# hynkis/Python-MPC

Measured on NVIDIA B200. Metric: lateral-MPC QP solves/sec (batch 65536, H=20), higher is better.
Workload: dtype f64

## Files before the change

### python-mpc_b200/csrc/mpc_b200.cu

```cuda
#include "shape_ops.cuh"
#include "models.cuh"

static thread_local std::string g_err;
static int env_int(const char* name, int dflt) { const char* v = std::getenv(name); return v ? std::atoi(v) : dflt; }
namespace mpcb_rt {
std::atomic<long long> g_launches{0};
std::atomic<int> g_opt_tma{std::getenv("MPCB_NO_TMA") ? 0 : 1};
std::atomic<int> g_opt_retile{std::getenv("MPCB_NO_RETILE") ? 0 : 1};
std::atomic<int> g_opt_cert{std::getenv("MPCB_NO_CERT") ? 0 : 1};
std::atomic<int> g_opt_dense{std::getenv("MPCB_NO_DENSE") ? 0 : 1};
std::atomic<int> g_opt_cta{std::getenv("MPCB_NO_CTA") ? 0 : 1};
std::atomic<int> g_opt_warp_setup{std::getenv("MPCB_NO_WARP_SETUP") ? 0 : 1};
std::atomic<int> g_opt_retile_min{env_int("MPCB_RETILE_MIN_BATCH", 4096)};
std::atomic<int> g_opt_fwd_rhs{std::getenv("MPCB_NO_FWD_RHS") ? 0 : 1};
int fail(int code, const std::string& msg) {
    g_err = msg;
    return code;
}
}

static const ShapeOps** registry(int* count_out, const ShapeOps* add) {
    static const ShapeOps* table[64];
    static int count = 0;
    if (add && count < 64) table[count++] = add;
    if (count_out) *count_out = count;
    return table;
}
namespace mpcb_rt {
void register_shape_ops(const ShapeOps* ops) { registry(nullptr, ops); }
}
static const ShapeOps* find_ops(int nx, int nu, int slack, int dtype) {
    int n = 0;
    const ShapeOps** t = registry(&n, nullptr);
    for (int i = 0; i < n; ++i)
        if (t[i]->nx == nx && t[i]->nu == nu && (t[i]->slack != 0) == (slack != 0) && t[i]->dtype == dtype) return t[i];
    return nullptr;
}
static const ShapeOps* ops_of(const mpcb_solver* s) {
    return find_ops(s->prob.nx, s->prob.nu, s->prob.slack, s->prob.dtype);
}

static bool is_big(double v) { return !(std::fabs(v) < kOsqpInfty * kMinScaling * 1e-6); }
static int problem_has_inf_bounds(const mpcb_problem& q) {
    for (int i = 0; i < q.nx; ++i) if (is_big(q.xmin[i]) || is_big(q.xmax[i])) return 1;
    for (int i = 0; i < q.nu; ++i) if (is_big(q.umin[i]) || is_big(q.umax[i])) return 1;
    return 0;
}

static bool shape_supported(int nx, int nu, int slack) { return find_ops(nx, nu, slack, MPCB_F64) != nullptr; }


const char* mpcb_last_error(void) { return g_err.c_str(); }
int mpcb_version(void) { return 100; }
long long mpcb_launch_count(void) { return g_launches.load(); }

int mpcb_set_option(const char* name, int value) {
    if (!name) return fail(MPCB_E_ARG, "null option name");
    const std::string n(name);
    if (n == "tma") g_opt_tma = value != 0;
    else if (n == "retile") g_opt_retile = value != 0;
    else if (n == "certificates") g_opt_cert = value != 0;
    else if (n == "dense") g_opt_dense = value != 0;
    else if (n == "warp_setup") g_opt_warp_setup = value != 0;
    else if (n == "cta") g_opt_cta = value < 0 ? 0 : (value > 2 ? 2 : value);
    else if (n == "retile_min_batch") g_opt_retile_min = value;
    else if (n == "fwd_rhs") g_opt_fwd_rhs = value != 0;
    else return fail(MPCB_E_ARG, "unknown option: " + n);
    return 0;
}

void mpcb_default_settings(mpcb_settings* s) {
    s->rho = 0.1; s->sigma = 1e-6; s->alpha = 1.6; s->eps_abs = 1e-3; s->eps_rel = 1e-3;
    s->eps_prim_inf = 1e-4; s->eps_dual_inf = 1e-4; s->max_iter = 4000; s->scaling = 10;
    s->check_termination = 25; s->warm_start = 1;
}

static int check_settings(const mpcb_settings* o) {
    if (!(o->rho > 0) || !(o->sigma > 0) || !(o->alpha > 0 && o->alpha < 2) || o->max_iter <= 0 ||
        o->scaling < 0 || o->check_termination < 0 || o->eps_abs < 0 || o->eps_rel < 0 ||
        (o->eps_abs == 0 && o->eps_rel == 0))
        return fail(MPCB_E_ARG, "invalid settings (rho, sigma > 0; 0 < alpha < 2; max_iter > 0; eps >= 0, not both 0)");
    return 0;
}

int mpcb_create(const mpcb_problem* prob, const mpcb_settings* settings, int capacity, mpcb_solver** out) {
    if (!prob || !out || capacity <= 0) return fail(MPCB_E_ARG, "null problem / non-positive capacity");
    if (prob->horizon < 1) return fail(MPCB_E_ARG, "horizon must be >= 1");
    if (prob->dtype != MPCB_F32 && prob->dtype != MPCB_F64) return fail(MPCB_E_ARG, "dtype must be MPCB_F32 or MPCB_F64");
    if (!shape_supported(prob->nx, prob->nu, prob->slack))
        return fail(MPCB_E_ARG, "unsupported (nx, nu, slack) combination");
    for (int i = 0; i < prob->nx; ++i)
        if (prob->xmin[i] > prob->xmax[i]) return fail(MPCB_E_ARG, "lower bound must be lower than or equal to upper bound");
    for (int i = 0; i < prob->nu; ++i)
        if (prob->umin[i] > prob->umax[i]) return fail(MPCB_E_ARG, "lower bound must be lower than or equal to upper bound");
    mpcb_settings def;
    mpcb_default_settings(&def);
    if (!settings) settings = &def;
    if (int rc = check_settings(settings)) return rc;
    mpcb_solver* s = new (std::nothrow) mpcb_solver();
    if (!s) return fail(MPCB_E_ALLOC, "out of host memory");
    s->prob = *prob; s->set = *settings; s->cap = capacity;
#ifndef MPCB_EMU
    if (cudaGetDevice(&s->dev) != cudaSuccess ||
        cudaDeviceGetAttribute(&s->dev_max_smem, cudaDevAttrMaxSharedMemoryPerBlockOptin, s->dev) != cudaSuccess ||
        cudaDeviceGetAttribute(&s->dev_sms, cudaDevAttrMultiProcessorCount, s->dev) != cudaSuccess) {
        const std::string msg = std::string("cuda device query: ") + cudaGetErrorString(cudaGetLastError());
        delete s;
        return fail(MPCB_E_CUDA, msg);
    }
#endif
    s->inf_prob = problem_has_inf_bounds(*prob);
    s->inf_bounds = s->inf_prob;
    s->esz = prob->dtype == MPCB_F32 ? 4 : 8;
    const int N = prob->horizon, nx = prob->nx, nu = prob->nu, ns = prob->slack ? nx : 0;
    s->VS = nx + ns + nu; s->CS = 2 * nx + nu; s->NW = nx + nu; s->LT = s->NW * (s->NW + 1) / 2;
    s->REC = 2 * s->VS + 2 * s->CS + s->LT + s->NW; s->HDR = 3 * nx + 1;
    s->nvar = (N + 1) * nx + N * nu + (N + 1) * ns; s->ncon = 2 * (N + 1) * nx + N * nu;
    s->ld = ((size_t)capacity + 31) / 32 * 32;
    const size_t ld = s->ld, e = s->esz, S1 = (size_t)(N + 1);
    struct { void** p; size_t n; } allocs[] = {
        {&s->rec, S1 * s->REC * ld * e}, {&s->hdr, (size_t)s->HDR * ld * e}, {&s->yrows, S1 * s->CS * ld * e},
        {&s->scr, S1 * (s->VS + s->CS) * ld * e}, {&s->scr_hdr, (size_t)nx * ld * e}, {&s->pri, ld * e},
        {&s->dua, ld * e}, {(void**)&s->iter, ld * sizeof(int)}, {(void**)&s->status, ld * sizeof(int)},
        {(void**)&s->tile_counter, 64}, {(void**)&s->surv[0], ld * sizeof(int)}, {(void**)&s->surv[1], ld * sizeof(int)},
        {(void**)&s->n_surv, 64}, {(void**)&s->tile_prog, (ld / 32 + 1) * sizeof(int)}};
    for (auto& a : allocs) {
        if (int rc = rt_malloc(a.p, a.n)) { mpcb_destroy(s); return rc; }
        s->ws_bytes += a.n;
    }
    rt_memset(s->rec, 0, S1 * s->REC * ld * e, 0);
    rt_memset(s->hdr, 0, (size_t)s->HDR * ld * e, 0);
    rt_memset(s->yrows, 0, S1 * s->CS * ld * e, 0);
    rt_memset(s->status, 0, ld * sizeof(int), 0);
    rt_sync(0);
    *out = s;
    return 0;
}

void mpcb_destroy(mpcb_solver* s) {
    if (!s) return;
    void* ptrs[] = {s->rec, s->hdr, s->yrows, s->scr, s->scr_hdr, s->pri, s->dua, s->iter, s->status, s->tile_counter,
                    s->surv[0], s->surv[1], s->n_surv, s->tile_prog, s->rec2, s->hdr2, s->yrows2,
                    s->xbox, s->xbox_alt, s->stage_in, s->stage_out, s->soa_in, s->dense_minv, s->dense_flag, s->mdl, s->mdl2};
    for (void* p : ptrs) rt_free(p);
    delete s;
}

int mpcb_set_settings(mpcb_solver* s, const mpcb_settings* o) {
    if (!s || !o) return fail(MPCB_E_ARG, "null argument");
// ... 470 lines not shown
```

### python-mpc_b200/csrc/qp_thread.cuh

```cuda
#pragma once
#include "mpc_common.h"

namespace mpcb {

MPCB_HD float msqrt(float v) { return sqrtf(v); }
MPCB_HD double msqrt(double v) { return sqrt(v); }
template <typename T> MPCB_HD T tmax(T a, T b) { return a > b ? a : b; }
template <typename T> MPCB_HD T tmin(T a, T b) { return a < b ? a : b; }
template <typename T> MPCB_HD T tabs(T a) { return a < (T)0 ? -a : a; }
template <typename T> MPCB_HD T limit_scaling(T v) {
    v = v < (T)kMinScaling ? (T)1 : v;
    return v > (T)kMaxScaling ? (T)kMaxScaling : v;
}
template <typename T> MPCB_HD T clip_infty(T v) {
    return tmin(tmax(v, (T)-kOsqpInfty), (T)kOsqpInfty);
}
template <typename T> MPCB_HD T row_rho(T l, T u, T rho, T rho_eq) {
    if (l < (T)(-kOsqpInfty * kMinScaling) && u > (T)(kOsqpInfty * kMinScaling)) return (T)kRhoMin;
    if (u - l < (T)kRhoTol) return rho_eq;
    return rho;
}
template <typename T> MPCB_HD T row_rho(bool inf_possible, T l, T u, T rho, T rho_eq) {
    if (inf_possible) return row_rho(l, u, rho, rho_eq);
    return (u - l < (T)kRhoTol) ? rho_eq : rho;
}
template <typename T> MPCB_HD T clamp_rho(T rho) {
    return tmin(tmax(rho, (T)kRhoMin), (T)kRhoMax);
}
MPCB_HD float fast_rcp(float v) { return 1.0f / v; }
MPCB_HD double fast_rcp(double v) {
#ifdef __CUDA_ARCH__
    double r;
    asm("rcp.approx.ftz.f64 %0, %1;" : "=d"(r) : "d"(v));
    r = r * (2.0 - v * r);
    r = r * (2.0 - v * r);
    return r;
#else
    return 1.0 / v;
#endif
}

MPCB_HD float fast_rsqrt(float v) { return 1.0f / sqrtf(v); }
MPCB_HD double fast_rsqrt(double v) {
#ifdef __CUDA_ARCH__
    double y;
    asm("rsqrt.approx.ftz.f64 %0, %1;" : "=d"(y) : "d"(v));
    double e = fma(-(v * y), y, 1.0);
    y = fma(0.5 * y, e, y);
    e = fma(-(v * y), y, 1.0);
    y = fma(0.5 * y, e, y);
    return y;
#else
    return 1.0 / sqrt(v);
#endif
}

template <typename T, typename L>
struct Model {
    T A[L::NX][L::NX];
    T B[L::NX][L::NU];
};
template <typename T, typename L>
MPCB_HD T model_g(const KParams<T>& p, int b, int k, int i) {
    if (!p.gd) return (T)0;
    const size_t og = p.tv ? (size_t)k * L::NX : 0;
    return p.model_bs ? p.gd[(og + i) * p.ld + b] : p.gd[og + i];
}

template <typename T, typename L>
MPCB_HD void load_model(const KParams<T>& p, int b, int k, Model<T, L>& m) {
    constexpr int NX = L::NX, NU = L::NU;
    const size_t bo = p.model_bs ? (size_t)b : 0;
    const size_t ld = p.model_bs ? p.ld : 1;
    const size_t oa = p.tv ? (size_t)k * NX * NX : 0, ob = p.tv ? (size_t)k * NX * NU : 0;
#pragma unroll
    for (int i = 0; i < NX; ++i) {
#pragma unroll
        for (int j = 0; j < NX; ++j) m.A[i][j] = p.Ad[(oa + i * NX + j) * ld + bo];
#pragma unroll
        for (int j = 0; j < NU; ++j) m.B[i][j] = p.Bd[(ob + i * NU + j) * ld + bo];
    }
}

template <typename T, typename L>
MPCB_HD void stage_box(const KParams<T>& p, int k, T* lo, T* hi) {
#pragma unroll
    for (int i = 0; i < L::NX; ++i) {
        T a = p.xbox ? p.xbox[(k * 2 + 0) * L::NX + i] : p.xmin[i];
        T c = p.xbox ? p.xbox[(k * 2 + 1) * L::NX + i] : p.xmax[i];
        lo[i] = a;
        hi[i] = c;
    }
}

template <typename T, typename L>
struct Ws {
    T* rec;
    T* hdr;
    T* y;
    T* scr;
    T* scr_hdr;
    MPCB_HD Ws(const KParams<T>& p, int b) {
        const size_t tile = (size_t)(b >> 5), lane = (size_t)(b & 31);
        const size_t S1 = (size_t)(p.N + 1);
        rec = p.rec + tile * S1 * L::REC * TILE + lane;
        hdr = p.hdr + tile * L::HDR * TILE + lane;
        y = p.yrows + tile * S1 * L::CS * TILE + lane;
        scr = p.scr + tile * S1 * (L::VS + L::CS) * TILE + lane;
        scr_hdr = p.scr_hdr + tile * L::NX * TILE + lane;
    }
    MPCB_HD T* R(int k) const { return rec + (size_t)k * L::REC * TILE; }
    MPCB_HD T* Y(int k) const { return y + (size_t)k * L::CS * TILE; }
    MPCB_HD T* S(int k) const { return scr + (size_t)k * (L::VS + L::CS) * TILE; }
};
#define MPCB_AT(ptr, e) (ptr)[(e) * TILE]

template <typename T, typename L>
struct ScaleStage {
    T Dx[L::NX], Dsl[L::NX], Du[L::NU], Ebx[L::NX], Ebu[L::NU], Edn[L::NX];
};
template <typename T, typename L>
MPCB_HD void scale_stage_update(const KParams<T>& p, const Model<T, L>& m, T c, int b, int k, const ScaleStage<T, L>& o,
                                const T* Ed_cur, const T* Dx_next, ScaleStage<T, L>& n, T* E0new, T& sumP, T& maxq) {
    constexpr int NX = L::NX, NU = L::NU, NS = L::NS;
    const bool last = (k == p.N);
    const T* Qk = last ? p.QN : p.Q;
    T colx[NX], colu[NU], rowd[NX];
#pragma unroll
    for (int j = 0; j < NX; ++j) {
        T v = c * tabs(Qk[j]) * o.Dx[j] * o.Dx[j];
        v = tmax(v, Ed_cur[j] * o.Dx[j]);
        colx[j] = tmax(v, o.Ebx[j] * o.Dx[j]);
        rowd[j] = o.Edn[j] * Dx_next[j];
    }
#pragma unroll
    for (int j = 0; j < NU; ++j) colu[j] = tmax(c * tabs(p.R[j]) * o.Du[j] * o.Du[j], o.Ebu[j] * o.Du[j]);
    if (!last) {
#pragma unroll
        for (int i = 0; i < NX; ++i) {
#pragma unroll
            for (int j = 0; j < NX; ++j) {
                const T gij = tabs(m.A[i][j]) * o.Edn[i] * o.Dx[j];
                colx[j] = tmax(colx[j], gij); rowd[i] = tmax(rowd[i], gij);
            }
#pragma unroll
            for (int j = 0; j < NU; ++j) {
                const T gij = tabs(m.B[i][j]) * o.Edn[i] * o.Du[j];
                colu[j] = tmax(colu[j], gij); rowd[i] = tmax(rowd[i], gij);
            }
        }
    }
#pragma unroll
    for (int j = 0; j < NX; ++j) {
        n.Dx[j] = o.Dx[j] * fast_rsqrt(limit_scaling(colx[j]));
        if (NS) {
            T w = tmax(c * tabs(p.W[j]) * o.Dsl[j] * o.Dsl[j], tabs(p.S[j]) * o.Ebx[j] * o.Dsl[j]);
            n.Dsl[j] = o.Dsl[j] * fast_rsqrt(limit_scaling(w));
        } else {
            n.Dsl[j] = (T)1;
        }
    }
#pragma unroll
    for (int j = 0; j < NU; ++j) n.Du[j] = last ? (T)1 : o.Du[j] * fast_rsqrt(limit_scaling(colu[j]));
    if (k == 0) {
#pragma unroll
        for (int i = 0; i < NX; ++i) {
            T v = Ed_cur[i] * o.Dx[i];
            E0new[i] = Ed_cur[i] * fast_rsqrt(limit_scaling(v));
        }
    }
#pragma unroll
    for (int i = 0; i < NX; ++i) {
        T en = (T)1;
        if (!last) en = o.Edn[i] * fast_rsqrt(limit_scaling(rowd[i]));
        n.Edn[i] = en;
        T w = o.Ebx[i] * o.Dx[i];
        if (NS) w = tmax(w, tabs(p.S[i]) * o.Ebx[i] * o.Dsl[i]);
        n.Ebx[i] = o.Ebx[i] * fast_rsqrt(limit_scaling(w));
    }
#pragma unroll
    for (int j = 0; j < NU; ++j) {
        T w = o.Ebu[j] * o.Du[j];
        n.Ebu[j] = last ? (T)1 : o.Ebu[j] * fast_rsqrt(limit_scaling(w));
    }
#pragma unroll
    for (int j = 0; j < NX; ++j) {
        sumP += c * tabs(Qk[j]) * n.Dx[j] * n.Dx[j];
        const T xr = p.Xr[((p.xr_tv ? (size_t)k * NX : 0) + j) * p.ld + b];
        maxq = tmax(maxq, tabs(c * n.Dx[j] * (-(Qk[j] * xr))));
        if (NS) sumP += c * tabs(p.W[j]) * n.Dsl[j] * n.Dsl[j];
    }
#pragma unroll
    for (int j = 0; j < NU; ++j)
        if (!last) sumP += c * tabs(p.R[j]) * n.Du[j] * n.Du[j];
}
template <typename T, typename L>
MPCB_HD T scale_cost_update(T c, T sumP, T maxq, int N) {
    T c_temp = sumP / (T)L::nvar(N);
    const T nq = limit_scaling(maxq);
    c_temp = tmax(c_temp, nq);
    c_temp = (T)1 / limit_scaling(c_temp);
    return c * c_temp;
}

template <typename T, typename L, bool ODD>
MPCB_HD void scale_pass(const KParams<T>& p, int b, const Ws<T, L>& ws, Model<T, L>& m, T& c) {
    constexpr int NX = L::NX, NU = L::NU, NS = L::NS;
    constexpr bool odd = ODD;
    const int N = p.N;
    const T* E0s = odd ? ws.scr_hdr : ws.hdr + L::H_E0 * TILE;
    T* E0d = odd ? ws.hdr + L::H_E0 * TILE : ws.scr_hdr;
    T sumP = 0, maxq = 0;
    T Ed_cur[NX];
#pragma unroll
    for (int i = 0; i < NX; ++i) Ed_cur[i] = MPCB_AT(E0s, i);
    for (int k = 0; k <= N; ++k) {
        const bool last = (k == N);
        const T* Ds = odd ? ws.S(k) : ws.R(k) + L::R_D * TILE;
        const T* Es = odd ? ws.S(k) + L::VS * TILE : ws.R(k) + L::R_E * TILE;
        T* Dd = odd ? ws.R(k) + L::R_D * TILE : ws.S(k);
        T* Ed = odd ? ws.R(k) + L::R_E * TILE : ws.S(k) + L::VS * TILE;
        const T* Dsn_ = last ? Ds : (odd ? ws.S(k + 1) : ws.R(k + 1) + L::R_D * TILE);
        if (p.tv && !last) load_model<T, L>(p, b, k, m);
        ScaleStage<T, L> o, n;
        T Dx_next[NX], E0new[NX];
#pragma unroll
        for (int i = 0; i < NX; ++i) {
            o.Dx[i] = MPCB_AT(Ds, L::OX + i);
            o.Dsl[i] = NS ? MPCB_AT(Ds, L::OS + (NS ? i : 0)) : (T)1;
            o.Ebx[i] = MPCB_AT(Es, L::OBX + i);
            o.Edn[i] = last ? (T)1 : MPCB_AT(Es, L::ODN + i);
            Dx_next[i] = last ? (T)1 : MPCB_AT(Dsn_, L::OX + i);
        }
#pragma unroll
        for (int j = 0; j < NU; ++j) {
            o.Du[j] = MPCB_AT(Ds, L::OU + j);
            o.Ebu[j] = MPCB_AT(Es, L::OBU + j);
        }
        scale_stage_update<T, L>(p, m, c, b, k, o, Ed_cur, Dx_next, n, E0new, sumP, maxq);
        if (k == 0) {
#pragma unroll
            for (int i = 0; i < NX; ++i) MPCB_AT(E0d, i) = E0new[i];
        }
#pragma unroll
        for (int i = 0; i < NX; ++i) {
            MPCB_AT(Ed, L::ODN + i) = n.Edn[i];
            MPCB_AT(Ed, L::OBX + i) = n.Ebx[i];
            MPCB_AT(Dd, L::OX + i) = n.Dx[i];
            if (NS) MPCB_AT(Dd, L::OS + (NS ? i : 0)) = n.Dsl[i];
        }
#pragma unroll
        for (int j = 0; j < NU; ++j) {
            MPCB_AT(Ed, L::OBU + j) = n.Ebu[j];
            MPCB_AT(Dd, L::OU + j) = n.Du[j];
        }
#pragma unroll
        for (int i = 0; i < NX; ++i) Ed_cur[i] = o.Edn[i];
    }
    c = scale_cost_update<T, L>(c, sumP, maxq, N);
}

template <typename T, typename L>
MPCB_HD void scale_one(const KParams<T>& p, int b) {
    constexpr int NX = L::NX;
    const int N = p.N;
    Ws<T, L> ws(p, b);
    for (int k = 0; k <= N; ++k) {
        T* R = ws.R(k);
        for (int e = 0; e < L::VS + L::CS; ++e) MPCB_AT(R, L::R_D + e) = (T)1;
    }
    for (int i = 0; i < NX; ++i) MPCB_AT(ws.hdr, L::H_E0 + i) = (T)1;
    T c = (T)1;
    Model<T, L> m;
    if (!p.tv) load_model<T, L>(p, b, 0, m);
    for (int it = 0; it < p.scaling; ++it) {
        if (it & 1) scale_pass<T, L, true>(p, b, ws, m, c);
        else scale_pass<T, L, false>(p, b, ws, m, c);
// ... 889 lines not shown
```

### python-mpc_b200/csrc/runtime.cuh

```cuda
#pragma once
#include "../../include/mpc_b200.h"
#include "mpc_common.h"
#include "qp_thread.cuh"

#include <atomic>
#include <cstdio>
#include <cstdlib>
#include <cstring>
#include <new>
#include <string>
#include <type_traits>

using namespace mpcb;

namespace mpcb_rt {
extern std::atomic<long long> g_launches;
extern std::atomic<int> g_opt_tma, g_opt_retile, g_opt_cert, g_opt_dense, g_opt_cta, g_opt_warp_setup, g_opt_retile_min, g_opt_fwd_rhs;
int fail(int code, const std::string& msg);
}
struct ShapeOps;
namespace mpcb_rt { void register_shape_ops(const ShapeOps* ops); }
using namespace mpcb_rt;

#ifndef MPCB_EMU
#include <cuda_runtime.h>
typedef cudaStream_t rt_stream;
#define RT_CHECK(expr)                                                                         \
    do {                                                                                       \
        cudaError_t e_ = (expr);                                                               \
        if (e_ != cudaSuccess)                                                                 \
            return fail(MPCB_E_CUDA, std::string(#expr) + ": " + cudaGetErrorString(e_));      \
    } while (0)
static int rt_malloc(void** p, size_t n) { RT_CHECK(cudaMalloc(p, n ? n : 1)); return 0; }
static void rt_free(void* p) { if (p) cudaFree(p); }
static int rt_memset(void* p, int v, size_t n, rt_stream s) { RT_CHECK(cudaMemsetAsync(p, v, n, s)); return 0; }
static int rt_h2d(void* d, const void* h, size_t n, rt_stream s) { RT_CHECK(cudaMemcpyAsync(d, h, n, cudaMemcpyHostToDevice, s)); return 0; }
static int rt_d2h(void* h, const void* d, size_t n, rt_stream s) { RT_CHECK(cudaMemcpyAsync(h, d, n, cudaMemcpyDeviceToHost, s)); return 0; }
static int rt_sync(rt_stream s) { RT_CHECK(cudaStreamSynchronize(s)); return 0; }
static bool debug_sync() {
    static const bool on = std::getenv("MPCB_DEBUG_SYNC") != nullptr;
    return on;
}
static int rt_launch_check(const char* what) {
    cudaError_t e = cudaGetLastError();
    if (e == cudaSuccess && debug_sync()) e = cudaDeviceSynchronize();
    if (e != cudaSuccess) return fail(MPCB_E_CUDA, std::string(what) + ": " + cudaGetErrorString(e));
    return 0;
}

#ifndef MPCB_QP_THREADS
#define MPCB_QP_THREADS 128
#endif
#ifndef MPCB_QP_MINBLOCKS
#define MPCB_QP_MINBLOCKS 2
#endif
template <typename Op, typename T, typename L>
__global__ void __launch_bounds__(MPCB_QP_THREADS, MPCB_QP_MINBLOCKS) qp_kernel(const KParams<T> p) {
    const int b = blockIdx.x * blockDim.x + threadIdx.x;
    if (b < p.B) Op::template run<T, L>(p, b);
}
template <typename Op, typename T, typename L>
static int launch_qp(const KParams<T>& p, rt_stream st) {
    const int threads = MPCB_QP_THREADS;
    qp_kernel<Op, T, L><<<(p.B + threads - 1) / threads, threads, 0, st>>>(p);
    ++g_launches;
    return rt_launch_check(Op::name());
}
template <typename F>
__global__ void __launch_bounds__(128) lambda_kernel(int n, F f) {
    const int b = blockIdx.x * blockDim.x + threadIdx.x;
    if (b < n) f(b);
}
#define MPCB_LAMBDA [=] __device__
template <typename F>
static int launch_1d(int n, rt_stream st, F f) {
    if (n <= 0) return 0;
    lambda_kernel<<<(n + 127) / 128, 128, 0, st>>>(n, f);
    ++g_launches;
    return rt_launch_check("lambda_kernel");
}
#else
typedef void* rt_stream;
static int rt_malloc(void** p, size_t n) { *p = std::malloc(n ? n : 1); return *p ? 0 : fail(MPCB_E_ALLOC, "malloc"); }
static void rt_free(void* p) { std::free(p); }
static int rt_memset(void* p, int v, size_t n, rt_stream) { std::memset(p, v, n); return 0; }
static int rt_h2d(void* d, const void* h, size_t n, rt_stream) { std::memcpy(d, h, n); return 0; }
static int rt_d2h(void* h, const void* d, size_t n, rt_stream) { std::memcpy(h, d, n); return 0; }
static int rt_sync(rt_stream) { return 0; }
template <typename Op, typename T, typename L>
static int launch_qp(const KParams<T>& p, rt_stream) {
    for (int b = 0; b < p.B; ++b) Op::template run<T, L>(p, b);
    ++g_launches;
    return 0;
}
#define MPCB_LAMBDA [=]
template <typename F>
static int launch_1d(int n, rt_stream, F f) {
    for (int b = 0; b < n; ++b) f(b);
    ++g_launches;
    return 0;
// ... 74 lines not shown
```

### python-mpc_b200/csrc/setup_warp.cuh

```cuda
#pragma once
#include "qp_thread.cuh"

#if defined(__CUDACC__) && !defined(MPCB_EMU)
namespace mpcb {

constexpr int SCALE_WARPS = 8;

template <typename T, typename L>
__global__ void __launch_bounds__(SCALE_WARPS * 32) scale_warp_kernel(const __grid_constant__ KParams<T> p) {
    constexpr int NX = L::NX, NU = L::NU, NS = L::NS;
    const int warp = threadIdx.x >> 5, k = threadIdx.x & 31;
    const int b = blockIdx.x * SCALE_WARPS + warp;
    if (b >= p.B) return;
    const int N = p.N;
    const bool stage = k <= N;
    const int kk = stage ? k : N;
    Model<T, L> m;
    load_model<T, L>(p, b, p.tv ? (kk < N ? kk : N - 1) : 0, m);
    ScaleStage<T, L> o, n;
    T E0[NX];
#pragma unroll
    for (int i = 0; i < NX; ++i) { o.Dx[i] = o.Dsl[i] = o.Ebx[i] = o.Edn[i] = (T)1; E0[i] = (T)1; }
#pragma unroll
    for (int j = 0; j < NU; ++j) { o.Du[j] = o.Ebu[j] = (T)1; }
    T c = (T)1;
    for (int it = 0; it < p.scaling; ++it) {
        T Ed_cur[NX], Dx_next[NX], E0new[NX];
#pragma unroll
        for (int i = 0; i < NX; ++i) {
            const T up = __shfl_up_sync(0xffffffffu, o.Edn[i], 1), dn = __shfl_down_sync(0xffffffffu, o.Dx[i], 1);
            Ed_cur[i] = k == 0 ? E0[i] : up;
            Dx_next[i] = k >= N ? (T)1 : dn;
            E0new[i] = E0[i];
        }
        T sumP = 0, maxq = 0;
        if (stage) scale_stage_update<T, L>(p, m, c, b, k, o, Ed_cur, Dx_next, n, E0new, sumP, maxq);
#pragma unroll
        for (int off = 16; off > 0; off >>= 1) {
            sumP += __shfl_xor_sync(0xffffffffu, sumP, off);
            maxq = tmax(maxq, __shfl_xor_sync(0xffffffffu, maxq, off));
        }
        c = scale_cost_update<T, L>(c, sumP, maxq, N);
        if (stage) o = n;
#pragma unroll
        for (int i = 0; i < NX; ++i) E0[i] = E0new[i];
    }
    if (!stage) return;
    Ws<T, L> ws(p, b);
    T* R = ws.R(k);
#pragma unroll
    for (int i = 0; i < NX; ++i) {
        MPCB_AT(R, L::R_D + L::OX + i) = o.Dx[i];
        if (NS) MPCB_AT(R, L::R_D + L::OS + (NS ? i : 0)) = o.Dsl[i];
        MPCB_AT(R, L::R_E + L::ODN + i) = o.Edn[i];
        MPCB_AT(R, L::R_E + L::OBX + i) = o.Ebx[i];
        if (k == 0) MPCB_AT(ws.hdr, L::H_E0 + i) = E0[i];
    }
#pragma unroll
    for (int j = 0; j < NU; ++j) {
        MPCB_AT(R, L::R_D + L::OU + j) = o.Du[j];
        MPCB_AT(R, L::R_E + L::OBU + j) = o.Ebu[j];
    }
    if (k == 0) MPCB_AT(ws.hdr, L::H_C) = c;
}

}
#endif
```

### python-mpc_b200/csrc/shape_ops.cuh

```cuda
#pragma once
#include <chrono>
#include "runtime.cuh"
#include "admm_kernel.cuh"
#include "admm_dense.cuh"
#include "admm_cta.cuh"
#include "setup_warp.cuh"

struct BuildOut {
    void *Pdiag, *q, *Avals, *l, *u;
};

struct ShapeOps {
    int nx, nu, slack, dtype;
    int (*setup)(mpcb_solver* s, rt_stream st);
    int (*refactor)(mpcb_solver* s, const mpcb_problem* np, void* new_box, rt_stream st);
    int (*run_admm)(mpcb_solver* s, int max_iter, int check_every, int warm, rt_stream st);
    int (*cold_start)(mpcb_solver* s, rt_stream st);
    int (*build_qp)(mpcb_solver* s, const BuildOut* o, rt_stream st);
};

struct ScaleOp { static const char* name() { return "scale"; } template <typename T, typename L> static MPCB_HD void run(const KParams<T>& p, int b) { scale_one<T, L>(p, b); } };
struct FactorOp { static const char* name() { return "factor"; } template <typename T, typename L> static MPCB_HD void run(const KParams<T>& p, int b) { factor_one<T, L>(p, b); } };
struct AdmmOp { static const char* name() { return "admm"; } template <typename T, typename L> static MPCB_HD void run(const KParams<T>& p, int b) { admm_one<T, L>(p, b); } };
struct ColdOp { static const char* name() { return "cold_start"; } template <typename T, typename L> static MPCB_HD void run(const KParams<T>& p, int b) { Ws<T, L> ws(p, b); admm_cold_start<T, L>(p, ws); } };
// ... 498 lines not shown
        }
    }
    if (p.tv && s->mdl && s->mdl_dirty) {
        if (int r = tile_model<T, L>(s, p, st)) return r;
    }
    s->mdl_dirty = false;
    const bool use_cta = cta_planned<T, L>(s, B, p.tv != 0, check_every) && cta_applicable<T, L>(s, p);
    if (int r = ensure_factor_form<T, L>(s, p, use_cta, st)) return r;
    if (use_cta) {
        const bool cta_chunked = !no_retile && check_every < max_iter && B >= retile_min;
        const int rc = run_cta_loop<T, L>(s, p, max_iter, check_every, cta_chunked, st);
        if (rc <= 0) return rc < 0 ? (int)MPCB_E_CUDA : 0;
    }
    if (!chunked) {
        p.it0 = 0; p.it_stop = max_iter; p.list_survivors = 0;
        return launch_admm<T, L>(p, s, st);
    }
    const int rt_slot = warm ? 1 : 0;
    int it0 = 0;
    LoopSet<T, L> set{B};
    const bool trace = std::getenv("MPCB_TRACE") != nullptr;
    const auto t_start = std::chrono::steady_clock::now();
    auto trace_ms = [&]() {
        rt_sync(st);
        return std::chrono::duration<double, std::milli>(std::chrono::steady_clock::now() - t_start).count();
    };
    bool learnt_now = false;
    while (it0 < max_iter) {
        int stop = it0 + check_every;
        if (it0 == 0 && s->retile_at[rt_slot] > 0) stop = s->retile_at[rt_slot];
        p.B = set.n; p.survivors = s->surv[set.which]; p.qp_map = set.map;
        p.it0 = it0; p.it_stop = stop < max_iter ? stop : max_iter; p.list_survivors = 1;
        if (int r = launch_admm<T, L>(p, s, st)) return r;
        if (trace) std::fprintf(stderr, "[mpcb] admm %d..%d n=%d scratch=%d  t=%.3f ms\n", p.it0 + 1, p.it_stop, set.n, (int)(set.map != nullptr), trace_ms());
        it0 = p.it_stop;
        int n_unc = 0;
        if (int r = rt_d2h(&n_unc, s->n_surv, sizeof(int), st)) return r;
        if (int r = rt_sync(st)) return r;
        if (int r = rt_memset(s->n_surv, 0, sizeof(int), st)) return r;
        if (n_unc == 0 || it0 >= max_iter) {
            if (!set.map && !learnt_now && n_unc == 0) {
                int& at = s->retile_at[rt_slot];
                int& backoff = s->retile_backoff[rt_slot];
                if (at == it0 && it0 > check_every && backoff == 0) at = it0 - check_every;
                else if (at == 0) at = it0;
                if (backoff > 0) --backoff;
            }
            break;
        }
#ifndef MPCB_EMU
        const bool tail_cta = !p.tv && cta_planned<T, L>(s, n_unc, false, check_every) && cta_applicable<T, L>(s, p);
#else
        const bool tail_cta = false;
#endif
        if (tail_cta || (5 * n_unc <= 4 * set.n && set.n >= (retile_min < 1024 ? retile_min : 1024))) {
            if (!learnt_now) { s->retile_at[rt_slot] = it0; learnt_now = true; }
            if (int r = set.compact(s, p, n_unc, 0, st)) return r;
#ifndef MPCB_EMU
            if (tail_cta) {
                if (int r = launch_1d(set.n * (p.N + 1), st, MinvFromLinvFn<T, L>{p.rec, p.N + 1, set.n})) return r;
                KParams<T> pc = p;
                pc.minv = 1; pc.B = set.n; pc.qp_map = set.map; pc.survivors = s->surv[set.which];
                pc.it0 = it0; pc.it_stop = max_iter; pc.list_survivors = 0;
                const int rc = launch_cta<T, L>(pc, s, st);
                if (rc < 0) return (int)MPCB_E_CUDA;
                if (trace) std::fprintf(stderr, "[mpcb] cta %d..%d n=%d scratch=1 (stragglers)  t=%.3f ms\n", it0 + 1, max_iter, set.n, trace_ms());
                if (rc == 0) break;
            }
#endif
        } else if (!set.map && !learnt_now && it0 == s->retile_at[rt_slot]) {
            s->retile_at[rt_slot] = 0;
            s->retile_backoff[rt_slot] = 16;
        }
    }
    return set.copy_home(s, st);
}

template <typename T, typename L>
static int setup_impl(mpcb_solver* s, rt_stream st) {
    KParams<T> p = make_params<T>(s);
    if (int r = rt_memset(s->status, 0, s->ld * sizeof(int), st)) return r;
#ifndef MPCB_EMU
    if (p.N + 1 <= 32 && g_opt_warp_setup.load() != 0) {
        scale_warp_kernel<T, L><<<(p.B + SCALE_WARPS - 1) / SCALE_WARPS, SCALE_WARPS * 32, 0, st>>>(p);
        ++g_launches;
        if (int r = rt_launch_check("scale_warp")) return r;
    } else
#endif
    if (int r = launch_qp<ScaleOp, T, L>(p, st)) return r;
#ifndef MPCB_EMU
    s->rec_minv = cta_planned<T, L>(s, p.B, p.tv != 0, s->set.check_termination) && cta_fits<T, L>(s, p.tv != 0) &&
                  !dense_candidate<T, L>(s);
#else
    s->rec_minv = false;
#endif
    p.minv = s->rec_minv ? 1 : 0;
    if (int r = launch_qp<FactorOp, T, L>(p, st)) return r;
    s->mdl_dirty = false;
    if (p.tv && g_opt_cta.load() != 0) return tile_model<T, L>(s, p, st);
    return 0;
}
template <typename T, typename L>
static int refactor_impl(mpcb_solver* s, const mpcb_problem* np, void* new_box, rt_stream st) {
    RefactorFn<T, L> fn;
    fn.po = make_params<T>(s);
    const mpcb_problem keep = s->prob;
    void* keep_box = s->xbox;
    s->prob = *np; s->xbox = new_box;
    fn.pn = make_params<T>(s);
    s->prob = keep; s->xbox = keep_box;
    return launch_1d(fn.pn.B, st, fn);
}
template <typename T, typename L>
static int cold_impl(mpcb_solver* s, rt_stream st) {
    KParams<T> p = make_params<T>(s);
    return launch_qp<ColdOp, T, L>(p, st);
}
template <typename T, typename L>
static int build_impl(mpcb_solver* s, const BuildOut* o, rt_stream st) {
    KParams<T> p = make_params<T>(s);
    return launch_1d(p.B, st, BuildFn<T, L>{p, *o});
}
template <typename T, typename L>
static ShapeOps make_shape_ops() {
    ShapeOps o;
    o.nx = L::NX; o.nu = L::NU; o.slack = L::SLACK ? 1 : 0;
    o.dtype = std::is_same<T, float>::value ? MPCB_F32 : MPCB_F64;
    o.setup = &setup_impl<T, L>; o.refactor = &refactor_impl<T, L>; o.run_admm = &run_admm_impl<T, L>;
    o.cold_start = &cold_impl<T, L>; o.build_qp = &build_impl<T, L>;
    return o;
}
```

Before: 2.849 million.

## Pack multiple QP instances per block in Ruiz scaling setup kernel

Adds a scale_pack_kernel that packs several batch instances (N+1 stage threads each) into a 64-thread block and exchanges neighbour scaling factors through shared memory. The old kernel gave each instance its own 32-lane warp, so for H=20 about a third of the lanes sat idle. The new kernel also caches the reference trajectory in registers and adds an integer-compare path for abs, max and clamp in the scaling loop. In exchange it adds per-iteration block-wide syncs, a serial cost reduction done by a lead thread per instance, and bit tricks that assume the compared values are non-negative.

```diff
diff --git a/python-mpc_b200/csrc/mpc_b200.cu b/python-mpc_b200/csrc/mpc_b200.cu
--- a/python-mpc_b200/csrc/mpc_b200.cu
+++ b/python-mpc_b200/csrc/mpc_b200.cu
@@ -13,6 +13,7 @@
 std::atomic<int> g_opt_warp_setup{std::getenv("MPCB_NO_WARP_SETUP") ? 0 : 1};
 std::atomic<int> g_opt_retile_min{env_int("MPCB_RETILE_MIN_BATCH", 4096)};
 std::atomic<int> g_opt_fwd_rhs{std::getenv("MPCB_NO_FWD_RHS") ? 0 : 1};
+std::atomic<int> g_opt_setup_pack{std::getenv("MPCB_NO_SETUP_PACK") ? 0 : 1};
 int fail(int code, const std::string& msg) {
     g_err = msg;
     return code;
@@ -65,6 +66,7 @@
     else if (n == "cta") g_opt_cta = value < 0 ? 0 : (value > 2 ? 2 : value);
     else if (n == "retile_min_batch") g_opt_retile_min = value;
     else if (n == "fwd_rhs") g_opt_fwd_rhs = value != 0;
+    else if (n == "setup_pack") g_opt_setup_pack = value != 0;
     else return fail(MPCB_E_ARG, "unknown option: " + n);
     return 0;
 }
diff --git a/python-mpc_b200/csrc/qp_thread.cuh b/python-mpc_b200/csrc/qp_thread.cuh
--- a/python-mpc_b200/csrc/qp_thread.cuh
+++ b/python-mpc_b200/csrc/qp_thread.cuh
@@ -1,4 +1,6 @@
 #pragma once
+#include <string.h>
+#include <type_traits>
 #include "mpc_common.h"
 
 namespace mpcb {
@@ -11,6 +13,40 @@
 template <typename T> MPCB_HD T limit_scaling(T v) {
     v = v < (T)kMinScaling ? (T)1 : v;
     return v > (T)kMaxScaling ? (T)kMaxScaling : v;
+}
+MPCB_HD long long ord_bits(double v) {
+#ifdef __CUDA_ARCH__
+    return __double_as_longlong(v);
+#else
+    long long r; memcpy(&r, &v, sizeof r); return r;
+#endif
+}
+MPCB_HD int ord_bits(float v) {
+#ifdef __CUDA_ARCH__
+    return __float_as_int(v);
+#else
+    int r; memcpy(&r, &v, sizeof r); return r;
+#endif
+}
+MPCB_HD float mabs(float v) { return fabsf(v); }
+MPCB_HD double mabs(double v) { return fabs(v); }
+template <bool IC, typename T> MPCB_HD T rabs(T a) {
+    if constexpr (IC) return mabs(a); else return tabs(a);
+}
+template <bool IC, typename T> MPCB_HD T rmax(T a, T b) {
+    if constexpr (IC) return ord_bits(a) > ord_bits(b) ? a : b; else return tmax(a, b);
+}
+template <bool IC, typename T> MPCB_HD T rlimit(T v) {
+    if constexpr (IC) {
+        using I = decltype(ord_bits(v));
+        using U = typename std::make_unsigned<I>::type;
+        const I lo = ord_bits((T)kMinScaling), hi = ord_bits((T)kMaxScaling), inf = ord_bits((T)INFINITY);
+        const I bv = ord_bits(v);
+        v = bv < lo ? (T)1 : v;
+        return (U)bv - (U)hi - 1u < (U)inf - (U)hi ? (T)kMaxScaling : v;
+    } else {
+        return limit_scaling(v);
+    }
 }
 template <typename T> MPCB_HD T clip_infty(T v) {
     return tmin(tmax(v, (T)-kOsqpInfty), (T)kOsqpInfty);
@@ -119,80 +155,81 @@
 struct ScaleStage {
     T Dx[L::NX], Dsl[L::NX], Du[L::NU], Ebx[L::NX], Ebu[L::NU], Edn[L::NX];
 };
-template <typename T, typename L>
+template <typename T, typename L, bool IC = false>
 MPCB_HD void scale_stage_update(const KParams<T>& p, const Model<T, L>& m, T c, int b, int k, const ScaleStage<T, L>& o,
-                                const T* Ed_cur, const T* Dx_next, ScaleStage<T, L>& n, T* E0new, T& sumP, T& maxq) {
+                                const T* Ed_cur, const T* Dx_next, ScaleStage<T, L>& n, T* E0new, T& sumP, T& maxq,
+                                const T* xr = nullptr) {
     constexpr int NX = L::NX, NU = L::NU, NS = L::NS;
     const bool last = (k == p.N);
     const T* Qk = last ? p.QN : p.Q;
     T colx[NX], colu[NU], rowd[NX];
 #pragma unroll
     for (int j = 0; j < NX; ++j) {
-        T v = c * tabs(Qk[j]) * o.Dx[j] * o.Dx[j];
-        v = tmax(v, Ed_cur[j] * o.Dx[j]);
-        colx[j] = tmax(v, o.Ebx[j] * o.Dx[j]);
+        T v = c * rabs<IC>(Qk[j]) * o.Dx[j] * o.Dx[j];
+        v = rmax<IC>(v, Ed_cur[j] * o.Dx[j]);
+        colx[j] = rmax<IC>(v, o.Ebx[j] * o.Dx[j]);
         rowd[j] = o.Edn[j] * Dx_next[j];
     }
 #pragma unroll
-    for (int j = 0; j < NU; ++j) colu[j] = tmax(c * tabs(p.R[j]) * o.Du[j] * o.Du[j], o.Ebu[j] * o.Du[j]);
+    for (int j = 0; j < NU; ++j) colu[j] = rmax<IC>(c * rabs<IC>(p.R[j]) * o.Du[j] * o.Du[j], o.Ebu[j] * o.Du[j]);
     if (!last) {
 #pragma unroll
         for (int i = 0; i < NX; ++i) {
 #pragma unroll
             for (int j = 0; j < NX; ++j) {
-                const T gij = tabs(m.A[i][j]) * o.Edn[i] * o.Dx[j];
-                colx[j] = tmax(colx[j], gij); rowd[i] = tmax(rowd[i], gij);
+                const T gij = rabs<IC>(m.A[i][j]) * o.Edn[i] * o.Dx[j];
+                colx[j] = rmax<IC>(colx[j], gij); rowd[i] = rmax<IC>(rowd[i], gij);
             }
 #pragma unroll
             for (int j = 0; j < NU; ++j) {
-                const T gij = tabs(m.B[i][j]) * o.Edn[i] * o.Du[j];
-                colu[j] = tmax(colu[j], gij); rowd[i] = tmax(rowd[i], gij);
+                const T gij = rabs<IC>(m.B[i][j]) * o.Edn[i] * o.Du[j];
+                colu[j] = rmax<IC>(colu[j], gij); rowd[i] = rmax<IC>(rowd[i], gij);
             }
         }
     }
 #pragma unroll
     for (int j = 0; j < NX; ++j) {
-        n.Dx[j] = o.Dx[j] * fast_rsqrt(limit_scaling(colx[j]));
+        n.Dx[j] = o.Dx[j] * fast_rsqrt(rlimit<IC>(colx[j]));
         if (NS) {
-            T w = tmax(c * tabs(p.W[j]) * o.Dsl[j] * o.Dsl[j], tabs(p.S[j]) * o.Ebx[j] * o.Dsl[j]);
-            n.Dsl[j] = o.Dsl[j] * fast_rsqrt(limit_scaling(w));
+            T w = rmax<IC>(c * rabs<IC>(p.W[j]) * o.Dsl[j] * o.Dsl[j], rabs<IC>(p.S[j]) * o.Ebx[j] * o.Dsl[j]);
+            n.Dsl[j] = o.Dsl[j] * fast_rsqrt(rlimit<IC>(w));
         } else {
             n.Dsl[j] = (T)1;
         }
     }
 #pragma unroll
-    for (int j = 0; j < NU; ++j) n.Du[j] = last ? (T)1 : o.Du[j] * fast_rsqrt(limit_scaling(colu[j]));
+    for (int j = 0; j < NU; ++j) n.Du[j] = last ? (T)1 : o.Du[j] * fast_rsqrt(rlimit<IC>(colu[j]));
     if (k == 0) {
 #pragma unroll
         for (int i = 0; i < NX; ++i) {
             T v = Ed_cur[i] * o.Dx[i];
-            E0new[i] = Ed_cur[i] * fast_rsqrt(limit_scaling(v));
+            E0new[i] = Ed_cur[i] * fast_rsqrt(rlimit<IC>(v));
         }
     }
 #pragma unroll
     for (int i = 0; i < NX; ++i) {
         T en = (T)1;
-        if (!last) en = o.Edn[i] * fast_rsqrt(limit_scaling(rowd[i]));
+        if (!last) en = o.Edn[i] * fast_rsqrt(rlimit<IC>(rowd[i]));
         n.Edn[i] = en;
         T w = o.Ebx[i] * o.Dx[i];
-        if (NS) w = tmax(w, tabs(p.S[i]) * o.Ebx[i] * o.Dsl[i]);
-        n.Ebx[i] = o.Ebx[i] * fast_rsqrt(limit_scaling(w));
+        if (NS) w = rmax<IC>(w, rabs<IC>(p.S[i]) * o.Ebx[i] * o.Dsl[i]);
+        n.Ebx[i] = o.Ebx[i] * fast_rsqrt(rlimit<IC>(w));
     }
 #pragma unroll
     for (int j = 0; j < NU; ++j) {
         T w = o.Ebu[j] * o.Du[j];
-        n.Ebu[j] = last ? (T)1 : o.Ebu[j] * fast_rsqrt(limit_scaling(w));
+        n.Ebu[j] = last ? (T)1 : o.Ebu[j] * fast_rsqrt(rlimit<IC>(w));
     }
 #pragma unroll
     for (int j = 0; j < NX; ++j) {
-        sumP += c * tabs(Qk[j]) * n.Dx[j] * n.Dx[j];
-        const T xr = p.Xr[((p.xr_tv ? (size_t)k * NX : 0) + j) * p.ld + b];
-        maxq = tmax(maxq, tabs(c * n.Dx[j] * (-(Qk[j] * xr))));
-        if (NS) sumP += c * tabs(p.W[j]) * n.Dsl[j] * n.Dsl[j];
+        sumP += c * rabs<IC>(Qk[j]) * n.Dx[j] * n.Dx[j];
+        const T xrj = xr ? xr[j] : p.Xr[((p.xr_tv ? (size_t)k * NX : 0) + j) * p.ld + b];
+        maxq = rmax<IC>(maxq, rabs<IC>(c * n.Dx[j] * (-(Qk[j] * xrj))));
+        if (NS) sumP += c * rabs<IC>(p.W[j]) * n.Dsl[j] * n.Dsl[j];
     }
 #pragma unroll
     for (int j = 0; j < NU; ++j)
-        if (!last) sumP += c * tabs(p.R[j]) * n.Du[j] * n.Du[j];
+        if (!last) sumP += c * rabs<IC>(p.R[j]) * n.Du[j] * n.Du[j];
 }
 template <typename T, typename L>
 MPCB_HD T scale_cost_update(T c, T sumP, T maxq, int N) {
diff --git a/python-mpc_b200/csrc/runtime.cuh b/python-mpc_b200/csrc/runtime.cuh
--- a/python-mpc_b200/csrc/runtime.cuh
+++ b/python-mpc_b200/csrc/runtime.cuh
@@ -15,7 +15,8 @@
 
 namespace mpcb_rt {
 extern std::atomic<long long> g_launches;
-extern std::atomic<int> g_opt_tma, g_opt_retile, g_opt_cert, g_opt_dense, g_opt_cta, g_opt_warp_setup, g_opt_retile_min, g_opt_fwd_rhs;
+extern std::atomic<int> g_opt_tma, g_opt_retile, g_opt_cert, g_opt_dense, g_opt_cta, g_opt_warp_setup, g_opt_retile_min, g_opt_fwd_rhs,
+    g_opt_setup_pack;
 int fail(int code, const std::string& msg);
 }
 struct ShapeOps;
diff --git a/python-mpc_b200/csrc/setup_warp.cuh b/python-mpc_b200/csrc/setup_warp.cuh
--- a/python-mpc_b200/csrc/setup_warp.cuh
+++ b/python-mpc_b200/csrc/setup_warp.cuh
@@ -64,5 +64,89 @@
     if (k == 0) MPCB_AT(ws.hdr, L::H_C) = c;
 }
 
+constexpr int SCALE_PACK_THREADS = 64;
+
+template <typename T, typename L>
+__global__ void __launch_bounds__(SCALE_PACK_THREADS) scale_pack_kernel(const __grid_constant__ KParams<T> p) {
+    constexpr int NX = L::NX, NU = L::NU, NS = L::NS, NT = SCALE_PACK_THREADS;
+    __shared__ T xEdn[NX][NT], xDx[NX][NT], rsum[NT], rmaxq[NT], cs[NT];
+    const int N = p.N, S1 = N + 1, Q = NT / S1;
+    const int t = threadIdx.x, q = t / S1, k = t - q * S1;
+    const int b = blockIdx.x * Q + q;
+    const bool stage = q < Q && b < p.B;
+    const int bl = blockIdx.x * Q + t;
+    const bool lead = t < Q && bl < p.B;
+    Model<T, L> m;
+    T xr[NX];
+    if (stage) {
+        load_model<T, L>(p, b, p.tv ? (k < N ? k : N - 1) : 0, m);
+#pragma unroll
+        for (int j = 0; j < NX; ++j) xr[j] = p.Xr[((p.xr_tv ? (size_t)k * NX : 0) + j) * p.ld + b];
+    }
+    if (lead) cs[t] = (T)1;
+    ScaleStage<T, L> o, n;
+    T E0[NX], Ed_cur[NX], Dx_next[NX];
+#pragma unroll
+    for (int i = 0; i < NX; ++i) { o.Dx[i] = o.Dsl[i] = o.Ebx[i] = o.Edn[i] = E0[i] = Ed_cur[i] = Dx_next[i] = (T)1; }
+#pragma unroll
+    for (int j = 0; j < NU; ++j) { o.Du[j] = o.Ebu[j] = (T)1; }
+    T c = (T)1;
+    for (int it = 0; it < p.scaling; ++it) {
+        if (stage) {
+            T E0new[NX];
+#pragma unroll
+            for (int i = 0; i < NX; ++i) E0new[i] = E0[i];
+            T sumP = 0, maxq = 0;
+            scale_stage_update<T, L, true>(p, m, c, b, k, o, Ed_cur, Dx_next, n, E0new, sumP, maxq, xr);
+            o = n;
+#pragma unroll
+            for (int i = 0; i < NX; ++i) { E0[i] = E0new[i]; xEdn[i][t] = o.Edn[i]; xDx[i][t] = o.Dx[i]; }
+            rsum[t] = sumP; rmaxq[t] = maxq;
+        }
+        __syncthreads();
+        if (stage) {
+#pragma unroll
+            for (int i = 0; i < NX; ++i) {
+                Ed_cur[i] = k == 0 ? E0[i] : xEdn[i][t - 1];
+                Dx_next[i] = k >= N ? (T)1 : xDx[i][t + 1];
+            }
+        }
+        if (lead) {
+            const int base = t * S1;
+            T s[16], mx[16];
+#pragma unroll
+            for (int v = 0; v < 16; ++v) {
+                const bool lo = v < S1, hi = v + 16 < S1;
+                s[v] = (lo ? rsum[base + v] : (T)0) + (hi ? rsum[base + v + 16] : (T)0);
+                mx[v] = rmax<true>(lo ? rmaxq[base + v] : (T)0, hi ? rmaxq[base + v + 16] : (T)0);
+            }
+#pragma unroll
+            for (int off = 8; off > 0; off >>= 1)
+#pragma unroll
+                for (int v = 0; v < off; ++v) { s[v] = s[v] + s[v + off]; mx[v] = rmax<true>(mx[v], mx[v + off]); }
+            cs[t] = scale_cost_update<T, L>(cs[t], s[0], mx[0], N);
+        }
+        __syncthreads();
+        if (stage) c = cs[q];
+    }
+    if (!stage) return;
+    Ws<T, L> ws(p, b);
+    T* R = ws.R(k);
+#pragma unroll
+    for (int i = 0; i < NX; ++i) {
+        MPCB_AT(R, L::R_D + L::OX + i) = o.Dx[i];
+        if (NS) MPCB_AT(R, L::R_D + L::OS + (NS ? i : 0)) = o.Dsl[i];
+        MPCB_AT(R, L::R_E + L::ODN + i) = o.Edn[i];
+        MPCB_AT(R, L::R_E + L::OBX + i) = o.Ebx[i];
+        if (k == 0) MPCB_AT(ws.hdr, L::H_E0 + i) = E0[i];
+    }
+#pragma unroll
+    for (int j = 0; j < NU; ++j) {
+        MPCB_AT(R, L::R_D + L::OU + j) = o.Du[j];
+        MPCB_AT(R, L::R_E + L::OBU + j) = o.Ebu[j];
+    }
+    if (k == 0) MPCB_AT(ws.hdr, L::H_C) = c;
+}
+
 }
 #endif
diff --git a/python-mpc_b200/csrc/shape_ops.cuh b/python-mpc_b200/csrc/shape_ops.cuh
--- a/python-mpc_b200/csrc/shape_ops.cuh
+++ b/python-mpc_b200/csrc/shape_ops.cuh
@@ -604,7 +604,12 @@
     if (int r = rt_memset(s->status, 0, s->ld * sizeof(int), st)) return r;
 #ifndef MPCB_EMU
     if (p.N + 1 <= 32 && g_opt_warp_setup.load() != 0) {
-        scale_warp_kernel<T, L><<<(p.B + SCALE_WARPS - 1) / SCALE_WARPS, SCALE_WARPS * 32, 0, st>>>(p);
+        if (g_opt_setup_pack.load() != 0) {
+            const int q = SCALE_PACK_THREADS / (p.N + 1);
+            scale_pack_kernel<T, L><<<(p.B + q - 1) / q, SCALE_PACK_THREADS, 0, st>>>(p);
+        } else {
+            scale_warp_kernel<T, L><<<(p.B + SCALE_WARPS - 1) / SCALE_WARPS, SCALE_WARPS * 32, 0, st>>>(p);
+        }
         ++g_launches;
         if (int r = rt_launch_check("scale_warp")) return r;
     } else
```

Result: faster. 2.906 million, median of 6 (+2.0%).

## Pack multiple QPs per CTA in scaling setup with shared-memory stage exchange

Applied to the files above, without the earlier changes.

Adds a scale_pack kernel that maps each horizon stage of several QPs onto threads of a 256-thread CTA. Neighbouring-stage scaling data and the per-iteration reductions are exchanged through double-buffered shared memory instead of warp-level exchange. The goal is to fill threads wasted when N+1 is below 32 in the warp-per-QP setup kernel and so speed up the Ruiz scaling phase. It uses much more shared memory per CTA, which can limit occupancy, and it only matters if setup is part of the timed solve.

```diff
diff --git a/python-mpc_b200/csrc/mpc_b200.cu b/python-mpc_b200/csrc/mpc_b200.cu
--- a/python-mpc_b200/csrc/mpc_b200.cu
+++ b/python-mpc_b200/csrc/mpc_b200.cu
@@ -13,6 +13,7 @@
 std::atomic<int> g_opt_warp_setup{std::getenv("MPCB_NO_WARP_SETUP") ? 0 : 1};
 std::atomic<int> g_opt_retile_min{env_int("MPCB_RETILE_MIN_BATCH", 4096)};
 std::atomic<int> g_opt_fwd_rhs{std::getenv("MPCB_NO_FWD_RHS") ? 0 : 1};
+std::atomic<int> g_opt_scale_pack{std::getenv("MPCB_NO_SCALE_PACK") ? 0 : 1};
 int fail(int code, const std::string& msg) {
     g_err = msg;
     return code;
@@ -65,6 +66,7 @@
     else if (n == "cta") g_opt_cta = value < 0 ? 0 : (value > 2 ? 2 : value);
     else if (n == "retile_min_batch") g_opt_retile_min = value;
     else if (n == "fwd_rhs") g_opt_fwd_rhs = value != 0;
+    else if (n == "scale_pack") g_opt_scale_pack = value < 0 ? 0 : (value > 2 ? 2 : value);
     else return fail(MPCB_E_ARG, "unknown option: " + n);
     return 0;
 }
diff --git a/python-mpc_b200/csrc/runtime.cuh b/python-mpc_b200/csrc/runtime.cuh
--- a/python-mpc_b200/csrc/runtime.cuh
+++ b/python-mpc_b200/csrc/runtime.cuh
@@ -15,7 +15,8 @@
 
 namespace mpcb_rt {
 extern std::atomic<long long> g_launches;
-extern std::atomic<int> g_opt_tma, g_opt_retile, g_opt_cert, g_opt_dense, g_opt_cta, g_opt_warp_setup, g_opt_retile_min, g_opt_fwd_rhs;
+extern std::atomic<int> g_opt_tma, g_opt_retile, g_opt_cert, g_opt_dense, g_opt_cta, g_opt_warp_setup, g_opt_retile_min, g_opt_fwd_rhs,
+    g_opt_scale_pack;
 int fail(int code, const std::string& msg);
 }
 struct ShapeOps;
diff --git a/python-mpc_b200/csrc/setup_warp.cuh b/python-mpc_b200/csrc/setup_warp.cuh
--- a/python-mpc_b200/csrc/setup_warp.cuh
+++ b/python-mpc_b200/csrc/setup_warp.cuh
@@ -64,5 +64,95 @@
     if (k == 0) MPCB_AT(ws.hdr, L::H_C) = c;
 }
 
+constexpr int SCALE_PACK_THREADS = 256;
+
+template <typename T, typename L>
+struct ScalePack {
+    static constexpr int SS = (int)(sizeof(ScaleStage<T, L>) / sizeof(T)) | 1;
+    static constexpr int MS = (int)(sizeof(Model<T, L>) / sizeof(T)) | 1;
+    static constexpr int MIN_CTAS = 2 * 2 * SCALE_PACK_THREADS * SS * sizeof(T) <= 192 * 1024 ? 2 : 1;
+    static int qps(int N) { return SCALE_PACK_THREADS / (N + 1); }
+    static size_t smem_bytes(int N, bool tv) {
+        return ((size_t)(2 * SS + 4) * SCALE_PACK_THREADS + (size_t)(2 * qps(N) + 1) * L::NX +
+                (size_t)(tv ? SCALE_PACK_THREADS : qps(N)) * MS) * sizeof(T);
+    }
+};
+
+template <typename T, int J, int STEP>
+__device__ __forceinline__ T scale_pack_sum(const T* s, int N) {
+    if constexpr (STEP == 32) return J <= N ? s[J] : (T)0;
+    else return scale_pack_sum<T, J, 2 * STEP>(s, N) + scale_pack_sum<T, J + STEP, 2 * STEP>(s, N);
+}
+
+template <typename T, typename L>
+__global__ void __launch_bounds__(SCALE_PACK_THREADS, (ScalePack<T, L>::MIN_CTAS)) scale_pack_kernel(const __grid_constant__ KParams<T> p) {
+    typedef ScaleStage<T, L> SS_;
+    typedef ScalePack<T, L> SP;
+    constexpr int NX = L::NX, NU = L::NU, NS = L::NS, TH = SCALE_PACK_THREADS, SS = SP::SS;
+    const int N = p.N, S1 = N + 1, t = threadIdx.x;
+    const int qpc = TH / S1, q = t / S1, k = t - q * S1;
+    extern __shared__ __align__(16) unsigned char scale_pack_smem[];
+    T* sc = reinterpret_cast<T*>(scale_pack_smem);
+    T* stat = sc + 2 * TH * SS;
+    T* e0 = stat + 4 * TH;
+    T* ones = e0 + 2 * qpc * NX;
+    T* mdl = ones + NX;
+    const int b = blockIdx.x * qpc + q;
+    const bool live = q < qpc && b < p.B;
+    const Model<T, L>& m = *reinterpret_cast<const Model<T, L>*>(mdl + (p.tv ? t : q) * SP::MS);
+    if (live && (p.tv || k == 0)) {
+        Model<T, L> mg;
+        load_model<T, L>(p, b, p.tv ? (k < N ? k : N - 1) : 0, mg);
+        *reinterpret_cast<Model<T, L>*>(mdl + (p.tv ? t : q) * SP::MS) = mg;
+    }
+    for (int e = 0; e < SS; ++e) sc[t * SS + e] = (T)1;
+    if (t < qpc)
+        for (int i = 0; i < NX; ++i) e0[t * NX + i] = (T)1;
+    if (t < NX) ones[t] = (T)1;
+    T c = (T)1;
+    __syncthreads();
+    for (int it = 0; it < p.scaling; ++it) {
+        const int cur = it & 1;
+        T* old = sc + cur * TH * SS;
+        T* st = stat + cur * 2 * TH;
+        if (live) {
+            const SS_& o = *reinterpret_cast<const SS_*>(old + t * SS);
+            SS_& n = *reinterpret_cast<SS_*>(sc + ((cur ^ 1) * TH + t) * SS);
+            const T* Ed_cur = k == 0 ? e0 + (cur * qpc + q) * NX : reinterpret_cast<const SS_*>(old + (t - 1) * SS)->Edn;
+            const T* Dx_next = k >= N ? ones : reinterpret_cast<const SS_*>(old + (t + 1) * SS)->Dx;
+            T sumP = 0, maxq = 0;
+            scale_stage_update<T, L>(p, m, c, b, k, o, Ed_cur, Dx_next, n, e0 + ((cur ^ 1) * qpc + q) * NX, sumP, maxq);
+            st[t] = sumP;
+            st[TH + t] = maxq;
+        }
+        __syncthreads();
+        if (live) {
+            const T* sq = st + TH + (t - k);
+            T maxq = 0;
+            for (int j = 0; j <= N; ++j) maxq = tmax(maxq, sq[j]);
+            c = scale_cost_update<T, L>(c, scale_pack_sum<T, 0, 1>(st + (t - k), N), maxq, N);
+        }
+    }
+    if (!live) return;
+    const SS_& o = *reinterpret_cast<const SS_*>(sc + ((p.scaling & 1) * TH + t) * SS);
+    const T* E0 = e0 + ((p.scaling & 1) * qpc + q) * NX;
+    Ws<T, L> ws(p, b);
+    T* R = ws.R(k);
+#pragma unroll
+    for (int i = 0; i < NX; ++i) {
+        MPCB_AT(R, L::R_D + L::OX + i) = o.Dx[i];
+        if (NS) MPCB_AT(R, L::R_D + L::OS + (NS ? i : 0)) = o.Dsl[i];
+        MPCB_AT(R, L::R_E + L::ODN + i) = o.Edn[i];
+        MPCB_AT(R, L::R_E + L::OBX + i) = o.Ebx[i];
+        if (k == 0) MPCB_AT(ws.hdr, L::H_E0 + i) = E0[i];
+    }
+#pragma unroll
+    for (int j = 0; j < NU; ++j) {
+        MPCB_AT(R, L::R_D + L::OU + j) = o.Du[j];
+        MPCB_AT(R, L::R_E + L::OBU + j) = o.Ebu[j];
+    }
+    if (k == 0) MPCB_AT(ws.hdr, L::H_C) = c;
+}
+
 }
 #endif
diff --git a/python-mpc_b200/csrc/shape_ops.cuh b/python-mpc_b200/csrc/shape_ops.cuh
--- a/python-mpc_b200/csrc/shape_ops.cuh
+++ b/python-mpc_b200/csrc/shape_ops.cuh
@@ -604,9 +604,20 @@
     if (int r = rt_memset(s->status, 0, s->ld * sizeof(int), st)) return r;
 #ifndef MPCB_EMU
     if (p.N + 1 <= 32 && g_opt_warp_setup.load() != 0) {
-        scale_warp_kernel<T, L><<<(p.B + SCALE_WARPS - 1) / SCALE_WARPS, SCALE_WARPS * 32, 0, st>>>(p);
-        ++g_launches;
-        if (int r = rt_launch_check("scale_warp")) return r;
+        const size_t smem = ScalePack<T, L>::smem_bytes(p.N, p.tv != 0);
+        const int qpc = ScalePack<T, L>::qps(p.N), ctas = (p.B + qpc - 1) / qpc, pack = g_opt_scale_pack.load();
+        if (pack != 0 && (pack == 2 || ctas >= s->dev_sms) && smem <= (size_t)s->dev_max_smem) {
+            RT_CHECK(cudaFuncSetAttribute(scale_pack_kernel<T, L>, cudaFuncAttributeMaxDynamicSharedMemorySize, (int)smem));
+            RT_CHECK(cudaFuncSetAttribute(scale_pack_kernel<T, L>, cudaFuncAttributePreferredSharedMemoryCarveout,
+                                          (int)cudaSharedmemCarveoutMaxShared));
+            scale_pack_kernel<T, L><<<ctas, SCALE_PACK_THREADS, smem, st>>>(p);
+            ++g_launches;
+            if (int r = rt_launch_check("scale_pack")) return r;
+        } else {
+            scale_warp_kernel<T, L><<<(p.B + SCALE_WARPS - 1) / SCALE_WARPS, SCALE_WARPS * 32, 0, st>>>(p);
+            ++g_launches;
+            if (int r = rt_launch_check("scale_warp")) return r;
+        }
     } else
 #endif
     if (int r = launch_qp<ScaleOp, T, L>(p, st)) return r;
```

Measured after the change: 2.863 million before, 2.905 million after, median of 6. +1.4%, better.
